# stoneMo/DeepAVFusion

Measured on AMD Instinct MI355X. Metric: AV-pairs/sec, DeepAVFusion ViT-B pre-training step (224px + 10s audio, image mask 0.75), higher is better.
Workload: dtype bf16; 1 GPU; AVMAE(DeepAVFusion base) fwd+bwd+allreduce+AdamW, B=64/GPU, 224x224 RGB + (128,640) log-mel, masks 0.75/0.8, fusion attn_ratio 0.25 mlp_ratio 1.0; global_batch=64, parallelism=dp1, graph=True

## Files before the change

deepavfusion_amd/_lib.py:

```python
from __future__ import annotations

import ctypes as C
import os

import torch

_HERE = os.path.dirname(os.path.abspath(__file__))
LIB_PATH = os.path.join(_HERE, 'libdavfusion_hip.so')

_p, _i, _l, _f, _sz = C.c_void_p, C.c_int, C.c_long, C.c_float, C.c_size_t

ABI_VERSION = 9

SIGNATURES = {
    'dav_abi_version': [],
    'dav_build_flags': [],
    'dav_last_error_string': [],
    'dav_tune': [_i, _i],
    'dav_gemm_nt_bf16': [_p, _p, _i, _i, _i, _i, _i, _p, _p, _i, _p, _i, _p, _i, _p, _p, _p, _i, _i, _p, _p, _i, _i, _i, _f, _i, _p],
    'dav_gemm_nt_ln_bf16': [_p, _p, _i, _i, _i, _i, _i, _p, _p, _i, _p, _i, _p, _i, _p, _p, _p, _i, _i, _p, _p, _i, _i, _i, _f, _i, _p, _p],
    'dav_ln_fold_grouped': [_p, _i, _p],
    'dav_rowstats_cast': [_p, _l, _i, _i, _i, _p, _p, _p],
    'dav_layernorm_bwd_twin': [_p, _l, _p, _i, _p, _l, _p, _i, _i, _i, _f, _p, _p, _p, _p,
                               _p, _l, _i, _p, _l, _p, _l,
# ... 51 lines not shown
    'dav_attn_bias_fwd_f32': [_p, _p, _p, _p, _p, _i, _i, _i, _i, _i, _i, _l, _i, _l, _i, _l, _i, _l, _i, _f, _p, _i, _i, _p],
    'dav_attn_bias_bwd_f32': [_p] * 10 + [_i] * 6 + [_l, _i] * 8 + [_f, _p, _i, _i, _p, _i, _p],
    'dav_attn_drop_fwd_f32': [_p, _p, _p, _p, _p, _i, _i, _i, _i, _i, _i, _l, _i, _l, _i, _l, _i, _l, _i, _f, _p, _i, _f, _p],
    'dav_attn_drop_bwd_f32': [_p] * 10 + [_i] * 6 + [_l, _i] * 8 + [_f, _p, _i, _f, _i, _p],
    'dav_patch_gather_f32': [_p, _i, _i, _i, _i, _i, _i, _p, _i, _p, _p],
    'dav_rows_gather_f32': [_p, _l, _i, _p, _i, _i, _i, _p, _l, _p],
    'dav_pair_expand_f32': [_p, _p, _i, _i, _i, _i, _p, _p],
    'dav_pair_reduce_f32': [_p, _i, _i, _i, _i, _p, _p, _p],
    'dav_patch_mse_bwd_f32': [_p, _p, _p, _p, _p, _p, _p, _i, _i, _i, _i, _p, _p],
    'dav_add_f32': [_p, _p, _p, _l, _p],
    'dav_logmel': [_p, _i, _i, _i, _i, _i, _p, _p, _p, _p, _p, _p, _f, _i, _i, _p, _p],
    'dav_log10_eps': [_p, _f, _l, _p, _p],
    'dav_mean_l2n_f32': [_p, _i, _i, _i, _l, _l, _p, _p],
    'dav_knn_topk_f32': [_p] * 6 + [_i, _i, _i, _i, _l, _l, _i, _i, _i, _p, _p, _p, _sz, _p],
    'dav_knn_topk_wide_f32': [_p] * 6 + [_i, _i, _i, _i, _l, _l, _i, _i, _i, _p, _p, _p, _sz, _p],
    'dav_knn_vote_f32': [_p, _p, _i, _i, _i, _i, _p, _p, _i, _i, _p, _i, _p, _p, _p],
    'dav_ap_auc_f64': [_p, _l, _i, _i, _i, _p, _l, _l, _p, _p, _p, _i, _p, _p, _p, _p, _sz, _p],
    'dav_frame_transform_u8': [_p, _i, _i, _i, _p, _i, _f, _f, _f, _f, _f, _f, _p, _p],
    'dav_wave_resample_tile': [_i, _i, _i],
    'dav_wave_resample': [_p, _i, _i, _i, _l, _p, _i, _i, _i, _p, _i, _p, _i, _l, _p],
    'dav_stft_c32': [_p, _i, _i, _l, _i, _i, _p, _p, _p, _p, _l, _p],
    'dav_istft_c32': [_p, _l, _i, _i, _i, _i, _p, _p, _p, _p, _l, _p],
    'dav_sep_mask_istft': [_p, _i, _i, _l, _p, _i, _i, _i, _i, _i, _p, _p, _p, _p, _p, _p, _p, _l, _p],
    'dav_batch_begin': [_i],
    'dav_batch_lane': [],
    'dav_batch_region': [_i],
    'dav_batch_skip': [_i],
    'dav_batch_suspend': [_i],
    'dav_batch_end': [],
    'dav_batch_abort': [],
    'dav_batch_stats': [_p, _p],
    'dav_adamw_flat': [_p, _p, _p, _p, _p, _l, _p, _p, _i, _f, _f, _f, _p, _f, _p, _i, _p, _p, _p],
    'dav_step_guard': [_p, _p, _p, _f, _f, _p, _p, _p],
    'dav_cast_transpose_grouped': [_p, _i, _p],
}

class DavLnReduce(C.Structure):
    _fields_ = [('workspace', C.c_void_p), ('dgamma', C.c_void_p), ('dbeta', C.c_void_p), ('rows', C.c_int), ('D', C.c_int)]


class DavNtLn(C.Structure):
    _fields_ = [('stats', C.c_void_p), ('stats2', C.c_void_p), ('A2', C.c_void_p), ('ln_c', C.c_void_p), ('eps', C.c_float),
                ('a_r0', C.c_int), ('a_r1', C.c_int), ('stats_out', C.c_void_p), ('twin_out', C.c_void_p), ('ld_twin', C.c_int)]


class DavLnFold(C.Structure):
# ... 76 lines not shown
```

deepavfusion_amd/autograd_bridge.py:

```python
from __future__ import annotations

import os

import torch

from . import engine as E
from . import ops
from .ops import F32


_SIDE_STREAMS = {}


def _streams(dev):
    main = torch.cuda.current_stream(dev)
    if os.environ.get('DAV_STREAMS', '1') == '0':
        return main, main, main
    key = dev.index if dev.index is not None else torch.cuda.current_device()
    if key not in _SIDE_STREAMS:
        _SIDE_STREAMS[key] = (torch.cuda.Stream(dev), torch.cuda.Stream(dev))
    sa, sf = _SIDE_STREAMS[key]
    return main, sa, sf


# ... 187 lines not shown


def encoder_bwd(enc, t, dxi_b=None, dxa_b=None, dxf_b=None, dxi32=None, dxa32=None, dxf32=None, layer_cb=None):
    with E.deferred_wgrads():
        _encoder_bwd(enc, t, dxi_b, dxa_b, dxf_b, dxi32, dxa32, dxf32, layer_cb)


def _encoder_bwd(enc, t, dxi_b, dxa_b, dxf_b, dxi32, dxa32, dxf32, layer_cb=None):
    B = t['B']
    dev = t['x_i'].device
    vis = _vis(enc)

    def final_norm(norm, x, st, dy_b, dy32):
        g = torch.empty_like(x)
        gb = torch.empty(x.shape, dtype=E.BF16, device=dev)
        if dy_b is None and dy32 is None:
            return g.zero_(), gb.zero_()
        E.ln_bwd(norm, None, x, B, st, dy_bf16=dy_b, dy_f32=dy32, dx1=g, dx1_bf16=gb)
        return g, gb
    g_i, g_ib = final_norm(vis.norm, t['x_i'], t['st_i'], dxi_b, dxi32)
    g_a, g_ab = final_norm(enc.audio.norm, t['x_a'], t['st_a'], dxa_b, dxa32)
    g_f, g_fb = final_norm(enc.fusion_norm, t['x_f'], t['st_f'], dxf_b, dxf32)
    blocks = list(zip(vis.blocks, enc.audio.blocks, enc.fusion_blocks))
    main, sa, sf = _streams(dev)
    batched = t['lanes']
    for l, ((bi, ba, fb), (ti, ta, tf)) in reversed(list(enumerate(zip(blocks, t['layers'])))):
        hold = (g_i, g_ib, g_a, g_ab, g_f, g_fb)
        if batched:
            dx_f = dx_i = dx_a = None
            lane_f = fb is not None and E.fusion_block_batchable(fb, tf.get('dp'), tf.get('dr')) and not E.FUSION_ON_STREAM
            if fb is not None and E.FUSION_ON_STREAM:
                sf.wait_stream(main)
                with torch.cuda.stream(sf):
                    dx_f, dx_i, dx_a = E.fusion_block_bwd(fb, tf, g_f, g_fb)
            elif fb is not None and not lane_f:
                dx_f, dx_i, dx_a = E.fusion_block_bwd(fb, tf, g_f, g_fb)
            idle = E.FUSION_IDLE_BWD if lane_f else 0
            with E.batch() as bt:
                bt.lane()
                st_i = E.block_bwd_head(bi, ti, g_i, g_ib, idle_before_attn=idle)
                bt.lane()
                st_a = E.block_bwd_head(ba, ta, g_a, g_ab, idle_before_attn=idle)
                if lane_f:
                    bt.lane()
                    dx_f, dx_i, dx_a = E.fusion_block_bwd(fb, tf, g_f, g_fb)
            acc = 1 if fb is not None else 0
# ... 13 lines not shown
            with torch.cuda.stream(sa):
                g_a, g_ab, _ = E.block_bwd(ba, ta, g_a, g_ab)
            g_i, g_ib, _ = E.block_bwd(bi, ti, g_i, g_ib)
            main.wait_stream(sa)
        else:
            sa.wait_stream(main)
            sf.wait_stream(main)
            with torch.cuda.stream(sf):
                dx_f, dx_i, dx_a = E.fusion_block_bwd(fb, tf, g_f, g_fb)
            with torch.cuda.stream(sa):
                g_a, g_ab, dxf_a = E.block_bwd(ba, ta, g_a, g_ab, dx_mod=dx_a, dx_mod_acc=1,
                                               before_ln1=lambda: sa.wait_stream(sf))
            g_i, g_ib, dx_f = E.block_bwd(bi, ti, g_i, g_ib, dx_fus=dx_f, dx_fus_acc=1, dx_mod=dx_i, dx_mod_acc=1,
                                          before_ln1=lambda: main.wait_stream(sf))
            main.wait_stream(sa)
            main.wait_stream(sf)
            if sa is main:
                g_f, g_fb = dx_f.add_(dxf_a), None
            elif _ADD_CAST and E.PRECISION != 'fp32' and dx_f.is_contiguous() and dxf_a.is_contiguous() and dx_f.numel() % 4 == 0:
                g_f, g_fb = ops.add_cast(dx_f, dxf_a)
            else:
                g_f, g_fb = dx_f + dxf_a, None
        del hold
        if E.wgrad_flush_due(l, len(blocks)):
            E.flush_wgrads()
        if layer_cb is not None and l > 0:
            layer_cb(l)
    E.patch_embed_bwd(vis, t['t_pi'], g_i, g_ib)
    E.patch_embed_bwd(enc.audio, t['t_pa'], g_a, g_ab)
    E.gbuf(enc.fusion_tokens).add_(g_f.sum(dim=0, keepdim=True))
    E._ready(enc.fusion_tokens)


class _EncoderFn(torch.autograd.Function):
    @staticmethod
    def forward(ctx, enc, image, audio, ik32, ak32, return_embs, need_tape, *params):
        ctx.set_materialize_grads(False)
        with E.ln_fuse_for(need_tape):
            _, f32s, embs, tape = encoder_fwd(enc, image, audio, ik32, ak32, want_f32=True, collect_embs=return_embs)
        ctx.enc, ctx.tape = enc, (tape if need_tape else None)
        B = image.shape[0]
        outs = [x.view(B, -1, x.shape[-1]) for x in f32s]
        flat_embs = [e for tri in embs for e in tri]
        ctx.mark_non_differentiable(*flat_embs)
        return (*outs, *flat_embs)

    @staticmethod
    def backward(ctx, gi, ga, gf, *_):
        if ctx.tape is None:
            raise RuntimeError('backward through DeepAVFusion.forward called without a saved tape')
        c = lambda g: None if g is None else g.contiguous().view(-1, g.shape[-1])
        encoder_bwd(ctx.enc, ctx.tape, dxi32=c(gi), dxa32=c(ga), dxf32=c(gf))
        ctx.tape = None
# ... 111 lines not shown

    @staticmethod
    def backward(ctx, g):
        with E.deferred_wgrads():
            dx_f, dx_i, dx_a = E.fusion_block_bwd(ctx.fb, ctx.tape, g.contiguous(), None)
        return (None, dx_f, dx_i, dx_a) + (None,) * ctx.np


def fusion_block(fb, xmm, xv, xa):
    c = lambda x: x.to(dtype=F32).contiguous()
    return _FusionBlockFn.apply(fb, c(xmm), c(xv), c(xa), *list(fb.parameters()))


def avmae_fwd(model, image, audio, noise_i, noise_a):
    with E.fold_scope(model):
        return _avmae_fwd(model, image, audio, noise_i, noise_a)


def _avmae_fwd(model, image, audio, noise_i, noise_a):
    enc = model.encoder
    B = image.shape[0]
    Li, La = model.image_gs[0] * model.image_gs[1], model.audio_gs[0] * model.audio_gs[1]
    nki, nka = int(Li * (1 - model.image_mask_ratio)), int(La * (1 - model.audio_mask_ratio))
    ik, im, ir, ik32, ir32 = ops.mask_build(noise_i, nki)
    ak, am, ar, ak32, ar32 = ops.mask_build(noise_a, nka)
    (xi_b, xa_b, xf_b), _, _, t_enc = encoder_fwd(enc, image, audio, ik32, ak32)
    nF = enc.fusion_tokens.shape[1]
    dec_i, dec_a = model.decoder('image'), model.decoder('audio')
    main, sa, _ = _streams(image.device)
    lanes = t_enc['lanes']
    if lanes:
        with E.batch() as bt:
            bt.lane()
            pred_i, t_di = E.decoder_fwd(dec_i, xi_b, xf_b, ir32, B, nki, nF)
            loss_i, t_li = E.loss_fwd(image, pred_i, im, model.image_norm_loss)
            bt.lane()
            pred_a, t_da = E.decoder_fwd(dec_a, xa_b, xf_b, ar32, B, nka, nF)
            loss_a, t_la = E.loss_fwd(audio, pred_a, am, model.audio_norm_loss)
    else:
        si = main
        sa.wait_stream(main)
        if si is not main:
            si.wait_stream(main)

        def chain(dec, x_b, r32, nk, target, mask, norm_loss):
            pred, t_d = yield from E.decoder_fwd_steps(dec, x_b, xf_b, r32, B, nk, nF)
            loss, t_l = E.loss_fwd(target, pred, mask, norm_loss)
            return pred, t_d, loss, t_l
# ... 42 lines not shown
                if g_p is not None:
                    dp = (dp.float() + g_p.reshape(dp.shape)).to(E.BF16)
                return (yield from E.decoder_bwd_steps(dec, t_d, dp, k32, B))
            (dxa_b, dxf_a), (dxi_b, dxf_i) = paired_steps(
                chain(dec_a, t['audio'], t['pred_a'], t['am'], t['t_la'], g_la, g_pa, t['t_da'], t['ak32']), sa,
                chain(dec_i, t['image'], t['pred_i'], t['im'], t['t_li'], g_li, g_pi, t['t_di'], t['ik32']), si, DEC_JOIN)
            main.wait_stream(sa)
            if si is not main:
                main.wait_stream(si)
            E.deferred_operands_to(main)
    else:
        sa.wait_stream(main)
        with torch.cuda.stream(sa), E.deferred_wgrads():
            dpa = E.loss_bwd(t['audio'], t['pred_a'], t['am'], t['t_la'], g_la)
            if g_pa is not None:
                dpa = (dpa.float() + g_pa.reshape(dpa.shape)).to(E.BF16)
            dxa_b, dxf_a = E.decoder_bwd(dec_a, t['t_da'], dpa, t['ak32'], B)
        with E.deferred_wgrads():
            dpi = E.loss_bwd(t['image'], t['pred_i'], t['im'], t['t_li'], g_li)
            if g_pi is not None:
                dpi = (dpi.float() + g_pi.reshape(dpi.shape)).to(E.BF16)
            dxi_b, dxf_i = E.decoder_bwd(dec_i, t['t_di'], dpi, t['ik32'], B)
        main.wait_stream(sa)
    dxf32 = dxf_i.float() + dxf_a.float()
    if layer_cb is not None:
        layer_cb(len(model.encoder.fusion_blocks))
    encoder_bwd(model.encoder, t['t_enc'], dxi_b=dxi_b, dxa_b=dxa_b, dxf32=dxf32, layer_cb=layer_cb)


class _AVMAEFn(torch.autograd.Function):
    @staticmethod
    def forward(ctx, model, image, audio, noise_i, noise_a, need_tape, *params):
        ctx.set_materialize_grads(False)
        with E.ln_fuse_for(need_tape):
            outs, tape, aux = avmae_fwd(model, image, audio, noise_i, noise_a)
        ctx.model, ctx.tape, ctx.np = model, (tape if need_tape else None), len(params)
        model._last_masks = aux
        return outs

    @staticmethod
    def backward(ctx, g_li, g_la, g_pi, g_pa):
        z = lambda g: g.contiguous() if g is not None else torch.zeros((), dtype=F32, device=ctx.tape['image'].device)
        avmae_bwd(ctx.model, ctx.tape, z(g_li), z(g_la), g_pi, g_pa)
        ctx.tape = None
        return (None,) * (6 + ctx.np)


# ... 13 lines not shown
```

deepavfusion_amd/engine.py:

```python
from __future__ import annotations

import os
from typing import Callable, Dict, List, NamedTuple, Optional

import torch

from . import ops
from .ops import F32

BF16 = torch.bfloat16
PRECISION = 'bf16'


def set_precision(p: str):
    global BF16, PRECISION
    if p not in ('bf16', 'fp32'):
        raise ValueError(p)
    PRECISION = p
    BF16 = torch.float32 if p == 'fp32' else torch.bfloat16

_GRAD_READY: Optional[Callable[[torch.nn.Parameter], None]] = None


def set_grad_ready_hook(fn: Optional[Callable[[torch.nn.Parameter], None]]):
    global _GRAD_READY
    _GRAD_READY = fn


def _ready(*params):
    if _GRAD_READY is not None:
        if _BATCH is not None:
            _BATCH.pending_ready.extend(params)
            return
        for p in params:
            if p is not None and p.requires_grad:
                _GRAD_READY(p)


_BATCH = None
BATCH_STATS = [0, 0]

BATCH_POLICY = {'1': 'on', '0': 'off'}.get(os.environ.get('DAV_BATCH', ''), 'auto')
LANE_MIN_ROWS = int(os.environ.get('DAV_LANE_MIN_ROWS', str(1 << 30)))
FUSION_ON_STREAM = os.environ.get('DAV_FUSION_STREAM', '1') != '0'


def set_batch_policy(policy: str):
    global BATCH_POLICY
    assert policy in ('on', 'off', 'auto')
    BATCH_POLICY = policy


def batching_allowed() -> bool:
    return BATCH_POLICY != 'off' and PRECISION == 'bf16'


def lanes_for(rows: int) -> bool:
    if not batching_allowed():
        return False
    return BATCH_POLICY == 'on' or rows >= LANE_MIN_ROWS


class batch:
    def __init__(self, auto_lanes: bool = False):
        self.auto_lanes = auto_lanes
        self.active = False
        self.pending_ready = []
# ... 1290 lines not shown
    A = _e((B * nk, K), BF16, img.device)
    ops.patch_gather(img, ids_keep32, nk, A, pt)
    Wb = wcache(pe.proj.weight)
    tok = _e((B, nk, D), F32, img.device)
    pos_by_id = ids_keep32 is not None and not clip
    if ln_fuse_ok(D) and K % 64 == 0:
        tw = (_e((B * nk, D), BF16, img.device), _e((B * nk, D // 64, 2), F32, img.device))
        ops.gemm_nt_ln(A, Wb, B * nk, D, K, prod=dict(stats_out=tw[1], twin_out=tw[0], ld_twin=D), bias=pe.proj.bias, res=vit.pos_embed,
                       ldres=D, res_rows=ids_keep32 if pos_by_id else None, res_rowmap=None if pos_by_id else (L, 0, 0), C_out=tok)
        tw_set(tok, *tw)
    else:
        ops.gemm_nt(A, Wb, B * nk, D, K, bias=pe.proj.bias, res=vit.pos_embed, ldres=D,
                    res_rows=ids_keep32 if pos_by_id else None, res_rowmap=None if pos_by_id else (L, 0, 0), C_out=tok)
    return tok, dict(A=A, nk=nk)


def patch_embed_bwd(vit, t, g, gb):
    pe = vit.patch_embed
    D = vit.embed_dim
    A = t['A']
    M, K = A.shape
    if gb is None:
        gb = to_bf16(g)
    ops.gemm_tn(gb, A, M, D, K, gbuf(pe.proj.weight).view(D, K), beta=1, bias_grad=gbuf(pe.proj.bias))
    _ready(pe.proj.weight, pe.proj.bias)


def drain(steps):
    try:
        while True:
            next(steps)
    except StopIteration as e:
        return e.value


def decoder_fwd(dec, x_b, xf_b, ids_restore32, B, nk, nF):
    return drain(decoder_fwd_steps(dec, x_b, xf_b, ids_restore32, B, nk, nF))


def decoder_fwd_steps(dec, x_b, xf_b, ids_restore32, B, nk, nF):
    L = ids_restore32.shape[1]
    Dd = dec.embed.weight.shape[0]
    dev = x_b.device
    emb = lin_fwd(dec.embed, x_b, B * nk)
    x = _e((B, nF + L, Dd), F32, dev)
    lin_fwd(dec.embed, xf_b, B * nF, out=x, c_rowmap=(nF, nF + L, 0))
# ... 16 lines not shown
        return pred.view(B, L, P), tape
    hN = _e((B * L, D_), BF16, dev)
    mean, rstd = _e((B * L,), F32, dev), _e((B * L,), F32, dev)
    xs = x.view(-1)[nF * Dd:]
    ops.layernorm_fwd(xs, (nF + L) * Dd, L, None, 0, 0, B, Dd, dec.norm.weight, dec.norm.bias, dec.norm.eps, hN, None, mean, rstd)
    pred = lin_fwd(dec.pred, hN, B * L)
    P = pred.shape[1]
    tape = dict(x_b=x_b, xf_b=xf_b, x_last=x, tapes=tapes, hN=hN, stN=(mean, rstd), ids_restore32=ids_restore32, nk=nk, nF=nF, L=L)
    return pred.view(B, L, P), tape


def decoder_bwd(dec, t, dpred_b, ids_keep32, B):
    return drain(decoder_bwd_steps(dec, t, dpred_b, ids_keep32, B))


def decoder_bwd_steps(dec, t, dpred_b, ids_keep32, B):
    nk, nF, L = t['nk'], t['nF'], t['L']
    Dd = dec.embed.weight.shape[0]
    dev = dpred_b.device
    fused = t.get('ln_fused', False)
    dhN = lin_bwd(dec.pred, dpred_b, None if fused else t['hN'], B * L, wgrad=not fused)
    g = _e((B, nF + L, Dd), F32, dev)
    gb = _e((B * (nF + L), Dd), BF16, dev)
    g[:, :nF].zero_()
    gb.view(B, nF + L, Dd)[:, :nF].zero_()
    if fused:
        xb, st = t['tw_last']
        hN = _e((B * L, Dd), BF16, dev)
        ops.layernorm_bwd_twin((xb, nF * Dd), (nF + L) * Dd, (st, nF * (Dd // 64) * 2), L, None, 0, None, 0, B, Dd, dec.norm.eps,
                               dhN, None, dec.norm.weight, dec.norm.bias,
                               (g, nF * Dd), (nF + L) * Dd, 0, None, 0, (gb, nF * Dd), (nF + L) * Dd,
                               h_out=hN, dgamma=gbuf(dec.norm.weight), dbeta=gbuf(dec.norm.bias))
        lin_wgrad(dec.pred, dpred_b, hN, B * L)
    else:
        xs = t['x_last'].view(-1)[nF * Dd:]
        ops.layernorm_bwd(xs, (nF + L) * Dd, L, None, 0, 0, B, Dd, dhN, None, dec.norm.weight, t['stN'][0], t['stN'][1],
                          g.view(-1)[nF * Dd:], (nF + L) * Dd, 0, None, 0, gb.view(-1)[nF * Dd:], (nF + L) * Dd,
                          None, 0, 0, None, 0, None, 0, gbuf(dec.norm.weight), gbuf(dec.norm.bias))
    _ready(dec.norm.weight, dec.norm.bias)
    swin = getattr(dec, 'arch', 'plain') == 'swin'
    yield
    for blk, bt in zip(reversed(list(dec.blocks)), reversed(t['tapes'])):
        if swin:
            g, gb = swin_block_bwd(blk, bt, g, gb)
        else:
            g, gb, _ = block_bwd(blk, bt, g, gb)
        yield
    d_emb = _e((B * nk, Dd), BF16, dev)
    d_embf = _e((B * nF, Dd), BF16, dev)
    ops.rows_gather_cast(g, (nF + L) * Dd, nF, ids_keep32, B, nk, Dd, d_emb)
    ops.rows_gather_cast(g, (nF + L) * Dd, 0, None, B, nF, Dd, d_embf)
    ops.unshuffle_bwd_reduce(g, (nF + L) * Dd, nF, t['ids_restore32'], B, L, nk, Dd, gbuf(dec.pos_embed), gbuf(dec.mask_token))
    _ready(dec.pos_embed, dec.mask_token)
    dx_b = lin_bwd(dec.embed, d_emb, t['x_b'], B * nk, final=False)
    dxf_b = lin_bwd(dec.embed, d_embf, t['xf_b'], B * nF)
    return dx_b, dxf_b


LOG2E = 1.4426950408889634


def swin_block_fwd(blk, x, nF):
    B, R, D = x.shape
    L, dev = R - nF, x.device
    heads, nW = blk.num_heads, blk.num_windows
    A = blk.attn.window_area
    N, hd, M, Mw = A + nF, D // heads, B * R, B * nW * (A + nF)
    h1, _, st1 = ln_fwd(blk.norm1, None, x, B)
    seq = _e((Mw, D), BF16, dev)
    ops.window_unfold(h1, blk.rows32, B, nW, A, nF, L, D, 1.0, seq)
    qkv = lin_fwd(blk.attn.qkv, seq, Mw, out_bf16=True)
    nb = nW if blk.attn_mask is not None else 1
    ld = (N + 31) // 32 * 32
    bias = _e((nb, heads, N, ld), F32, dev)
    ops.relpos_bias_build(blk.attn.relative_position_bias_table, blk.index32, blk.attn_mask, nb, heads, A, N, ld,
# ... 35 lines not shown
    ops.relpos_bias_bwd(dS, blk.index32, B * nW, heads, A, N, t['ld'], table.shape[0], gbuf(table))
    _ready(table)
    dseq = lin_bwd(blk.attn.qkv, dqkv, t['seq'], Mw, dx_bf16=False)
    dh1 = _e((M, D), F32, dev)
    ops.window_fold(dseq, blk.inv32, None, B, nW, A, nF, L, D, 1.0, dh1)
    dx = _e((B, R, D), F32, dev)
    dxb = _e((M, D), BF16, dev)
    ln_bwd(blk.norm1, None, x, B, t['st1'], dy_f32=dh1, dx1=dx, res1=g1, dx1_bf16=dxb)
    return dx, dxb


def loss_fwd(img, pred, mask, norm_pix):
    B, L = mask.shape
    dev = img.device
    lp, tm, tr = _e((B * L,), F32, dev), _e((B * L,), F32, dev), _e((B * L,), F32, dev)
    loss, msum = _e((1,), F32, dev), _e((1,), F32, dev)
    ops.patch_mse_fwd(img, pred, mask, norm_pix, lp, tm, tr, loss, msum)
    return loss.view(()), dict(tm=tm, tr=tr, msum=msum)


def loss_bwd(img, pred, mask, t, gout):
    B, L, P = pred.shape
    dpred = _e((B * L, P), BF16, img.device)
    ops.patch_mse_bwd(img, pred, mask, t['tm'], t['tr'], t['msum'], gout, dpred)
    return dpred
```

deepavfusion_amd/ops.py:

```python
from __future__ import annotations

import ctypes as C
from typing import Optional, Sequence

import torch

from . import _lib

BF16 = torch.bfloat16
F32 = torch.float32


def _stream():
    return torch.cuda.current_stream().cuda_stream


import threading

_TLS = threading.local()


def hold(*tensors):
    h = getattr(_TLS, 'hold', None)
    if h is not None:
# ... 409 lines not shown

def unshuffle_bwd_reduce(dx, dx_bs, row_off, ids_restore32, B, L, nk, D, dpos, dmask_token):
    lib = _lib.load()
    _lib.check(lib.dav_unshuffle_bwd_reduce(_ptr(dx), dx_bs, row_off, _ptr(ids_restore32), B, L, nk, D, _ptr(dpos),
                                            _ptr(dmask_token), _stream()), 'dav_unshuffle_bwd_reduce')


def patch_mse_fwd(img, pred, mask, norm_pix, loss_patch, tmean, trstd, loss, mask_sum):
    lib = _lib.load()
    B, Cc, H, W = img.shape
    _lib.check(lib.dav_patch_mse_fwd(_ptr(img), _ptr(pred), _ptr(mask), B, Cc, H, W, int(norm_pix), _ptr(loss_patch),
                                     _ptr(tmean), _ptr(trstd), _ptr(loss), _ptr(mask_sum), _stream()), 'dav_patch_mse_fwd')


def patch_mse_bwd(img, pred, mask, tmean, trstd, mask_sum, gout, dpred_bf16):
    lib = _lib.load()
    B, Cc, H, W = img.shape
    if dpred_bf16.dtype == F32:
        _lib.check(lib.dav_patch_mse_bwd_f32(_ptr(img), _ptr(pred), _ptr(mask), _ptr(tmean), _ptr(trstd), _ptr(mask_sum), _ptr(gout),
                                             B, Cc, H, W, _ptr(dpred_bf16), _stream()), 'dav_patch_mse_bwd_f32')
        return
    _lib.check(lib.dav_patch_mse_bwd(_ptr(img), _ptr(pred), _ptr(mask), _ptr(tmean), _ptr(trstd), _ptr(mask_sum), _ptr(gout),
                                     B, Cc, H, W, _ptr(dpred_bf16), _stream()), 'dav_patch_mse_bwd')


def pair_expand(Pv, Pa, B, nv, na, Wd, out):
    lib = _lib.load()
    if out.dtype == F32:
        _lib.check(lib.dav_pair_expand_f32(_ptr(Pv), _ptr(Pa), B, nv, na, Wd, _ptr(out), _stream()), 'dav_pair_expand_f32')
        return
    _lib.check(lib.dav_pair_expand(_ptr(Pv), _ptr(Pa), B, nv, na, Wd, _ptr(out), _stream()), 'dav_pair_expand')


def pair_reduce(d, B, nv, na, Wd, dPv, dPa):
    lib = _lib.load()
    if d.dtype == F32:
        _lib.check(lib.dav_pair_reduce_f32(_ptr(d), B, nv, na, Wd, _ptr(dPv), _ptr(dPa), _stream()), 'dav_pair_reduce_f32')
        return
    _lib.check(lib.dav_pair_reduce(_ptr(d), B, nv, na, Wd, _ptr(dPv), _ptr(dPa), _stream()), 'dav_pair_reduce')


def cast_bf16(x, y):
    lib = _lib.load()
    _lib.check(lib.dav_cast_bf16(_ptr(x), _ptr(y), x.numel(), _stream()), 'dav_cast_bf16')


# ... 379 lines not shown
```

include/dav_kernels.h:

```cpp
#ifndef DAV_KERNELS_H_
#define DAV_KERNELS_H_

#include <stddef.h>
#include <stdint.h>

#ifdef __HIPCC__
#include <hip/hip_runtime.h>
#else
typedef struct ihipStream_t* hipStream_t;
#endif

#ifdef __cplusplus
extern "C" {
#endif

#define DAV_ABI_VERSION 9
int dav_abi_version(void);
int dav_build_flags(void);
const char* dav_last_error_string(void);
int dav_tune(int knob, int value);

int dav_gemm_nt_bf16(const void* A, const void* B, int M, int N, int K, int lda, int ldb, const int* a_rowmap,
                     const float* bias, int act, const void* aux, int ldaux, const float* res, int ldres,
                     const int* res_rowmap, const int* res_rows, void* C, int ldc, int c_is_bf16, const int* c_rowmap,
// ... 195 lines not shown
int dav_attn_bias_bwd_f32(const float* Q, const float* K, const float* V, const float* O, const float* dO, const float* LSE,
                          float* Delta, float* dQ, float* dK, float* dV, int B, int H, int Nq, int Nk, int dqk, int dv, long q_bs,
                          int q_rs, long k_bs, int k_rs, long v_bs, int v_rs, long o_bs, int o_rs, long do_bs, int do_rs,
                          long dq_bs, int dq_rs, long dk_bs, int dk_rs, long dv_bs, int dv_rs, float scale, const float* bias,
                          int bias_nb, int bias_ld, float* dS, int part, hipStream_t stream);
int dav_attn_drop_fwd_f32(const float* Q, const float* K, const float* V, float* O, float* LSE, int B, int H, int Nq, int Nk,
                          int dqk, int dv, long q_bs, int q_rs, long k_bs, int k_rs, long v_bs, int v_rs, long o_bs, int o_rs,
                          float scale, const void* keep, int keep_ld, float keep_scale, hipStream_t stream);
int dav_attn_drop_bwd_f32(const float* Q, const float* K, const float* V, const float* O, const float* dO, const float* LSE,
                          float* Delta, float* dQ, float* dK, float* dV, int B, int H, int Nq, int Nk, int dqk, int dv, long q_bs,
                          int q_rs, long k_bs, int k_rs, long v_bs, int v_rs, long o_bs, int o_rs, long do_bs, int do_rs,
                          long dq_bs, int dq_rs, long dk_bs, int dk_rs, long dv_bs, int dv_rs, float scale, const void* keep,
                          int keep_ld, float keep_scale, int part, hipStream_t stream);
int dav_patch_gather_f32(const float* img, int B, int C, int T, int H, int W, int pt, const int* ids_keep32, int nk, float* A,
                         hipStream_t stream);
int dav_rows_gather_f32(const float* x, long x_bs, int row_off, const int* ids32, int B, int n, int D, float* out, long out_bs,
                        hipStream_t stream);
int dav_pair_expand_f32(const float* Pv, const float* Pa, int B, int nv, int na, int Wd, float* out, hipStream_t stream);
int dav_pair_reduce_f32(const float* d, int B, int nv, int na, int Wd, float* dPv, float* dPa, hipStream_t stream);
int dav_patch_mse_bwd_f32(const float* img, const float* pred, const float* mask, const float* tmean, const float* trstd,
                          const float* mask_sum, const float* gout, int B, int C, int H, int W, float* dpred, hipStream_t stream);
int dav_add_f32(const float* a, const float* b, float* out, long n, hipStream_t stream);

int dav_batch_begin(int auto_lanes);
int dav_batch_lane(void);
int dav_batch_region(int begin);
int dav_batch_skip(int steps);
int dav_batch_suspend(int on);
int dav_batch_end(void);
int dav_batch_abort(void);
int dav_batch_stats(int* recorded_ops, int* issued_launches);

#ifdef __cplusplus
}
#endif
#endif
```

Before: 2659 AV-pairs/s.

## Add fused seam kernels for masks, loss bwd, reductions, zeroing and patch-embed wgrad

Adds a set of small HIP kernels behind a DAV_SEAMS switch, on by default for bf16. Mask building for image and audio now runs as one launch. It also adds a vectorized loss gradient, a decoder unshuffle reduction with unrolled batch loads, a bf16+bf16→f32 add and a batch-sum accumulate for the fusion tokens. The zeroing of two rows becomes a single kernel, and the patch-embed backward moves into the layer loop as deferred wgrad. These target launch count and small memory-bound kernels around the main encoder/decoder. In exchange they add atomics and deferred wgrad ordering that could change numerics or the schedule.

```diff
diff --git a/deepavfusion_amd/_lib.py b/deepavfusion_amd/_lib.py
--- a/deepavfusion_amd/_lib.py
+++ b/deepavfusion_amd/_lib.py
@@ -97,6 +97,12 @@
     'dav_stft_c32': [_p, _i, _i, _l, _i, _i, _p, _p, _p, _p, _l, _p],
     'dav_istft_c32': [_p, _l, _i, _i, _i, _i, _p, _p, _p, _p, _l, _p],
     'dav_sep_mask_istft': [_p, _i, _i, _l, _p, _i, _i, _i, _i, _i, _p, _p, _p, _p, _p, _p, _p, _l, _p],
+    'dav_unshuffle_bwd_reduce2': [_p, _l, _i, _p, _i, _i, _i, _i, _p, _p, _p],
+    'dav_patch_mse_bwd2': [_p, _p, _p, _p, _p, _p, _p, _i, _i, _i, _i, _p, _p],
+    'dav_mask_build_pair': [_p, _i, _i, _i, _p, _p, _p, _p, _p] * 2 + [_p],
+    'dav_add2_bf16_f32': [_p, _p, _p, _l, _p],
+    'dav_batch_sum_acc': [_p, _l, _i, _l, _p, _p],
+    'dav_rows_zero_pair': [_p, _p, _i, _i, _i, _i, _p],
     'dav_batch_begin': [_i],
     'dav_batch_lane': [],
     'dav_batch_region': [_i],
diff --git a/deepavfusion_amd/autograd_bridge.py b/deepavfusion_amd/autograd_bridge.py
--- a/deepavfusion_amd/autograd_bridge.py
+++ b/deepavfusion_amd/autograd_bridge.py
@@ -233,6 +233,7 @@
     g_a, g_ab = final_norm(enc.audio.norm, t['x_a'], t['st_a'], dxa_b, dxa32)
     g_f, g_fb = final_norm(enc.fusion_norm, t['x_f'], t['st_f'], dxf_b, dxf32)
     blocks = list(zip(vis.blocks, enc.audio.blocks, enc.fusion_blocks))
+    pembed_queued = False
     main, sa, sf = _streams(dev)
     batched = t['lanes']
     for l, ((bi, ba, fb), (ti, ta, tf)) in reversed(list(enumerate(zip(blocks, t['layers'])))):
@@ -292,13 +293,22 @@
             else:
                 g_f, g_fb = dx_f + dxf_a, None
         del hold
+        if l == 0 and E.seam('pembed'):
+            E.patch_embed_bwd(vis, t['t_pi'], g_i, g_ib)
+            E.patch_embed_bwd(enc.audio, t['t_pa'], g_a, g_ab)
+            pembed_queued = True
         if E.wgrad_flush_due(l, len(blocks)):
             E.flush_wgrads()
         if layer_cb is not None and l > 0:
             layer_cb(l)
-    E.patch_embed_bwd(vis, t['t_pi'], g_i, g_ib)
-    E.patch_embed_bwd(enc.audio, t['t_pa'], g_a, g_ab)
-    E.gbuf(enc.fusion_tokens).add_(g_f.sum(dim=0, keepdim=True))
+    if not pembed_queued:
+        E.patch_embed_bwd(vis, t['t_pi'], g_i, g_ib)
+        E.patch_embed_bwd(enc.audio, t['t_pa'], g_a, g_ab)
+    ft = E.gbuf(enc.fusion_tokens)
+    if E.seam('fsum') and g_f.dtype == F32 and g_f.is_contiguous() and ft.is_contiguous() and ft.numel() % 4 == 0 and g_f.numel() == B * ft.numel():
+        ops.batch_sum_acc(g_f, ft.numel(), B, ft.numel(), ft)
+    else:
+        ft.add_(g_f.sum(dim=0, keepdim=True))
     E._ready(enc.fusion_tokens)
 
 
@@ -456,8 +466,11 @@
     B = image.shape[0]
     Li, La = model.image_gs[0] * model.image_gs[1], model.audio_gs[0] * model.audio_gs[1]
     nki, nka = int(Li * (1 - model.image_mask_ratio)), int(La * (1 - model.audio_mask_ratio))
-    ik, im, ir, ik32, ir32 = ops.mask_build(noise_i, nki)
-    ak, am, ar, ak32, ar32 = ops.mask_build(noise_a, nka)
+    if E.seam('mask'):
+        (ik, im, ir, ik32, ir32), (ak, am, ar, ak32, ar32) = ops.mask_build_pair(noise_i, nki, noise_a, nka)
+    else:
+        ik, im, ir, ik32, ir32 = ops.mask_build(noise_i, nki)
+        ak, am, ar, ak32, ar32 = ops.mask_build(noise_a, nka)
     (xi_b, xa_b, xf_b), _, _, t_enc = encoder_fwd(enc, image, audio, ik32, ak32)
     nF = enc.fusion_tokens.shape[1]
     dec_i, dec_a = model.decoder('image'), model.decoder('audio')
@@ -546,7 +559,11 @@
                 dpi = (dpi.float() + g_pi.reshape(dpi.shape)).to(E.BF16)
             dxi_b, dxf_i = E.decoder_bwd(dec_i, t['t_di'], dpi, t['ik32'], B)
         main.wait_stream(sa)
-    dxf32 = dxf_i.float() + dxf_a.float()
+    if (E.seam('add2') and dxf_i.dtype == E.BF16 and dxf_a.dtype == E.BF16 and dxf_i.is_contiguous() and dxf_a.is_contiguous()
+            and dxf_i.numel() % 4 == 0):
+        dxf32 = ops.add2_bf16_f32(dxf_i, dxf_a)
+    else:
+        dxf32 = dxf_i.float() + dxf_a.float()
     if layer_cb is not None:
         layer_cb(len(model.encoder.fusion_blocks))
     encoder_bwd(model.encoder, t['t_enc'], dxi_b=dxi_b, dxa_b=dxa_b, dxf32=dxf32, layer_cb=layer_cb)
diff --git a/deepavfusion_amd/csrc/step/seams.hip b/deepavfusion_amd/csrc/step/seams.hip
--- /dev/null
+++ b/deepavfusion_amd/csrc/step/seams.hip
@@ -0,0 +1,272 @@
+#include "common.h"
+#include "dav_kernels.h"
+
+namespace {
+
+__device__ __forceinline__ void add4(float4& s, const float4& v) { s.x += v.x; s.y += v.y; s.z += v.z; s.w += v.w; }
+
+constexpr int UB = 8;
+
+__global__ __launch_bounds__(256) void unshuffle_bwd_reduce2_kernel(const float* dx, long dx_bs, int row_off, const int* restore,
+                                                                    int B, int L, int nk, int D, float* dpos, float* dmask_token) {
+  __shared__ float4 part[4][64];
+  const int lane = threadIdx.x & 63, w = threadIdx.x >> 6;
+  const int nch = D >> 2;
+  const int c = blockIdx.x * 64 + lane;
+  const int r = blockIdx.y * 4 + w;
+  const bool live = r < L && c < nch;
+  float4 sp = float4{0.f, 0.f, 0.f, 0.f}, sm = sp;
+  if (live) {
+    const float4* src = reinterpret_cast<const float4*>(dx + (long)(row_off + r) * D) + c;
+    const long bs4 = dx_bs >> 2;
+    const int* rs = restore + r;
+    int b = 0;
+    for (; b + UB <= B; b += UB) {
+      float4 v[UB];
+      int j[UB];
+#pragma unroll
+      for (int u = 0; u < UB; ++u) { v[u] = src[(b + u) * bs4]; j[u] = rs[(long)(b + u) * L]; }
+#pragma unroll
+      for (int u = 0; u < UB; ++u) {
+        add4(sp, v[u]);
+        if (j[u] >= nk) add4(sm, v[u]);
+      }
+    }
+    for (; b < B; ++b) {
+      const float4 v = src[b * bs4];
+      add4(sp, v);
+      if (rs[(long)b * L] >= nk) add4(sm, v);
+    }
+    float4* dp = reinterpret_cast<float4*>(dpos + (long)r * D) + c;
+    float4 o = *dp;
+    add4(o, sp);
+    *dp = o;
+  }
+  part[w][lane] = sm;
+  __syncthreads();
+  if (w == 0 && c < nch) {
+    float4 t = part[0][lane];
+    add4(t, part[1][lane]); add4(t, part[2][lane]); add4(t, part[3][lane]);
+    float* dm = dmask_token + 4 * c;
+    unsafeAtomicAdd(dm + 0, t.x); unsafeAtomicAdd(dm + 1, t.y); unsafeAtomicAdd(dm + 2, t.z); unsafeAtomicAdd(dm + 3, t.w);
+  }
+}
+
+template <int C>
+__device__ __forceinline__ const float* patch_px(const float* img, int b, int l, int H, int W, int lane) {
+  const int gW = W >> 4, gy = l / gW, gx = l % gW;
+  return img + (((long)b * C) * H + gy * 16 + (lane >> 2)) * W + gx * 16 + (lane & 3) * 4;
+}
+
+template <int C>
+__global__ __launch_bounds__(256) void patch_mse_bwd2_kernel(const float* img, const float* pred, const float* mask, const float* tmean,
+                                                             const float* trstd, const float* mask_sum, const float* gout, int B, int H,
+                                                             int W, bf16_t* dpred) {
+  constexpr int P = 256 * C;
+  const int lane = threadIdx.x & 63;
+  const int gw = (blockIdx.x * blockDim.x + threadIdx.x) >> 6, nwaves = (gridDim.x * blockDim.x) >> 6;
+  const int L = (H >> 4) * (W >> 4), n = B * L;
+  const long plane = (long)H * W;
+  const float coef = (gout ? gout[0] : 1.f) * 2.f / (P * mask_sum[0]);
+  for (int row = gw; row < n; row += nwaves) {
+    const float m = mask[row] * coef;
+    uint2* dst = reinterpret_cast<uint2*>(dpred + (long)row * P + lane * 4 * C);
+    if (m == 0.f) {
+#pragma unroll
+      for (int k = 0; k < C; ++k) dst[k] = uint2{0u, 0u};
+      continue;
+    }
+    const float mean = tmean[row], rstd = trstd[row];
+    const float* tp = patch_px<C>(img, row / L, row % L, H, W, lane);
+    const float4* pp = reinterpret_cast<const float4*>(pred + (long)row * P + lane * 4 * C);
+    float4 t[C], p4[C];
+#pragma unroll
+    for (int c = 0; c < C; ++c) { t[c] = *reinterpret_cast<const float4*>(tp + c * plane); p4[c] = pp[c]; }
+    const float* p = reinterpret_cast<const float*>(p4);
+    float g[4 * C];
+#pragma unroll
+    for (int c = 0; c < C; ++c) {
+      const float tc[4] = {t[c].x, t[c].y, t[c].z, t[c].w};
+#pragma unroll
+      for (int j = 0; j < 4; ++j) g[j * C + c] = m * (p[j * C + c] - (tc[j] - mean) * rstd);
+    }
+#pragma unroll
+    for (int k = 0; k < C; ++k) dst[k] = uint2{pack2bf(g[4 * k], g[4 * k + 1]), pack2bf(g[4 * k + 2], g[4 * k + 3])};
+  }
+}
+
+struct MaskSide {
+  const float* noise;
+  int64_t* ids_keep;
+  int64_t* ids_restore;
+  float* mask;
+  int* ids_keep32;
+  int* ids_restore32;
+  int N, L, P, len_keep;
+};
+
+__global__ __launch_bounds__(1024) void mask_build_pair_kernel(MaskSide sa, MaskSide sb) {
+  extern __shared__ __attribute__((aligned(16))) char smem[];
+  const bool first = (int)blockIdx.x < sa.N;
+  const MaskSide& s = first ? sa : sb;
+  const int row = first ? blockIdx.x : blockIdx.x - sa.N;
+  const int L = s.L, P = s.P, len_keep = s.len_keep;
+  float* key = reinterpret_cast<float*>(smem);
+  int* idx = reinterpret_cast<int*>(smem + (size_t)P * 4);
+  const int tid = threadIdx.x, nt = blockDim.x;
+  for (int i = tid; i < P; i += nt) {
+    key[i] = i < L ? s.noise[(long)row * L + i] : __int_as_float(0x7f800000);
+    idx[i] = i;
+  }
+  __syncthreads();
+  for (int k = 2; k <= P; k <<= 1) {
+    for (int j = k >> 1; j > 0; j >>= 1) {
+      for (int i = tid; i < P; i += nt) {
+        const int ixj = i ^ j;
+        if (ixj > i) {
+          const float a = key[i], b = key[ixj];
+          const int ia = idx[i], ib = idx[ixj];
+          const bool a_gt_b = (a > b) || (a == b && ia > ib);
+          const bool up = (i & k) == 0;
+          if (a_gt_b == up) { key[i] = b; key[ixj] = a; idx[i] = ib; idx[ixj] = ia; }
+        }
+      }
+      __syncthreads();
+    }
+  }
+  for (int i = tid; i < L; i += nt) {
+    const int src = idx[i];
+    s.ids_restore[(long)row * L + src] = i;
+    s.ids_restore32[(long)row * L + src] = i;
+    s.mask[(long)row * L + src] = i < len_keep ? 0.f : 1.f;
+    if (i < len_keep) {
+      s.ids_keep[(long)row * len_keep + i] = src;
+      s.ids_keep32[(long)row * len_keep + i] = src;
+    }
+  }
+}
+
+__global__ __launch_bounds__(256) void add2_bf16_f32_kernel(const uint2* a, const uint2* b, float4* out, long n4) {
+  for (long i = (long)blockIdx.x * blockDim.x + threadIdx.x; i < n4; i += (long)gridDim.x * blockDim.x) {
+    const uint2 x = a[i], y = b[i];
+    out[i] = float4{__uint_as_float(x.x << 16) + __uint_as_float(y.x << 16),
+                    __uint_as_float(x.x & 0xffff0000u) + __uint_as_float(y.x & 0xffff0000u),
+                    __uint_as_float(x.y << 16) + __uint_as_float(y.y << 16),
+                    __uint_as_float(x.y & 0xffff0000u) + __uint_as_float(y.y & 0xffff0000u)};
+  }
+}
+
+__global__ __launch_bounds__(64) void batch_sum_acc_kernel(const float* x, long x_bs, int B, long n4, float* acc) {
+  const long i = (long)blockIdx.x * blockDim.x + threadIdx.x;
+  if (i >= n4) return;
+  const float4* src = reinterpret_cast<const float4*>(x) + i;
+  const long bs4 = x_bs >> 2;
+  float4 s = float4{0.f, 0.f, 0.f, 0.f};
+  int b = 0;
+  for (; b + UB <= B; b += UB) {
+    float4 v[UB];
+#pragma unroll
+    for (int u = 0; u < UB; ++u) v[u] = src[(b + u) * bs4];
+#pragma unroll
+    for (int u = 0; u < UB; ++u) add4(s, v[u]);
+  }
+  for (; b < B; ++b) add4(s, src[b * bs4]);
+  float4* dst = reinterpret_cast<float4*>(acc) + i;
+  float4 o = *dst;
+  add4(o, s);
+  *dst = o;
+}
+
+__global__ __launch_bounds__(256) void rows_zero_pair_kernel(float* g, void* gb, int B, long bs, long z) {
+  const long per = (z >> 2) + (z >> 3), total = (long)B * per;
+  for (long i = (long)blockIdx.x * blockDim.x + threadIdx.x; i < total; i += (long)gridDim.x * blockDim.x) {
+    const long b = i / per, k = i % per;
+    if (k < (z >> 2)) reinterpret_cast<float4*>(g + b * bs)[k] = float4{0.f, 0.f, 0.f, 0.f};
+    else reinterpret_cast<uint4*>((bf16_t*)gb + b * bs)[k - (z >> 2)] = uint4{0u, 0u, 0u, 0u};
+  }
+}
+
+int wave_grid(long rows) {
+  long g = (rows + 3) / 4;
+  return (int)(g > 2048 ? 2048 : (g < 1 ? 1 : g));
+}
+
+int flat_grid(long items) {
+  long g = (items + 255) / 256;
+  return (int)(g > 4096 ? 4096 : (g < 1 ? 1 : g));
+}
+
+bool mis(const void* p, unsigned mask) { return ((uintptr_t)p & mask) != 0; }
+
+int mask_side(MaskSide& s, const float* noise, int N, int L, int len_keep, int64_t* ids_keep, int64_t* ids_restore, float* mask,
+              int* ids_keep32, int* ids_restore32) {
+  if (N <= 0 || L <= 0 || L > 4096 || len_keep < 0 || len_keep > L) return DAV_ERR_SHAPE;
+  int P = 1;
+  while (P < L) P <<= 1;
+  s = MaskSide{noise, ids_keep, ids_restore, mask, ids_keep32, ids_restore32, N, L, P, len_keep};
+  return DAV_OK;
+}
+
+}
+
+extern "C" int dav_unshuffle_bwd_reduce2(const float* dx, long dx_bs, int row_off, const int* ids_restore32, int B, int L, int nk,
+                                         int D, float* dpos, float* dmask_token, hipStream_t stream) {
+  if (B <= 0 || L <= 0 || D <= 0 || (D & 3) || row_off < 0 || dx_bs < 0) return DAV_ERR_SHAPE;
+  if ((dx_bs & 3) || mis(dx, 15) || mis(dpos, 15) || mis(dmask_token, 15) || mis(ids_restore32, 3)) return DAV_ERR_ALIGN;
+  const dim3 grid(((D >> 2) + 63) / 64, (L + 3) / 4);
+  DAV_LAUNCH(unshuffle_bwd_reduce2_kernel, grid, dim3(256), 0, stream, dx, dx_bs, row_off, ids_restore32, B, L, nk, D, dpos, dmask_token);
+  return dav_launch_status();
+}
+
+extern "C" int dav_patch_mse_bwd2(const float* img, const float* pred, const float* mask, const float* tmean, const float* trstd,
+                                  const float* mask_sum, const float* gout, int B, int C, int H, int W, void* dpred_bf16,
+                                  hipStream_t stream) {
+  if (B <= 0 || H <= 0 || W <= 0 || (H & 15) || (W & 15) || (C != 1 && C != 3)) return DAV_ERR_SHAPE;
+  const long rows = (long)B * (H >> 4) * (W >> 4);
+  if (rows > 0x7fffffffL) return DAV_ERR_SHAPE;
+  if (mis(img, 15) || mis(pred, 15) || mis(dpred_bf16, 7)) return DAV_ERR_ALIGN;
+  const dim3 grid(wave_grid(rows)), block(256);
+  if (C == 3) DAV_LAUNCH(patch_mse_bwd2_kernel<3>, grid, block, 0, stream, img, pred, mask, tmean, trstd, mask_sum, gout, B, H, W, (bf16_t*)dpred_bf16);
+  else DAV_LAUNCH(patch_mse_bwd2_kernel<1>, grid, block, 0, stream, img, pred, mask, tmean, trstd, mask_sum, gout, B, H, W, (bf16_t*)dpred_bf16);
+  return dav_launch_status();
+}
+
+extern "C" int dav_mask_build_pair(const float* noise_a, int Na, int La, int len_keep_a, int64_t* ids_keep_a, int64_t* ids_restore_a,
+                                   float* mask_a, int* ids_keep32_a, int* ids_restore32_a, const float* noise_b, int Nb, int Lb,
+                                   int len_keep_b, int64_t* ids_keep_b, int64_t* ids_restore_b, float* mask_b, int* ids_keep32_b,
+                                   int* ids_restore32_b, hipStream_t stream) {
+  MaskSide sa, sb;
+  if (mask_side(sa, noise_a, Na, La, len_keep_a, ids_keep_a, ids_restore_a, mask_a, ids_keep32_a, ids_restore32_a) != DAV_OK ||
+      mask_side(sb, noise_b, Nb, Lb, len_keep_b, ids_keep_b, ids_restore_b, mask_b, ids_keep32_b, ids_restore32_b) != DAV_OK)
+    return DAV_ERR_SHAPE;
+  const int P = sa.P > sb.P ? sa.P : sb.P;
+  const int nt = P / 2 < 64 ? 64 : (P / 2 > 1024 ? 1024 : P / 2);
+  DAV_LAUNCH(mask_build_pair_kernel, dim3(Na + Nb), dim3(nt), (size_t)P * 8, stream, sa, sb);
+  return dav_launch_status();
+}
+
+extern "C" int dav_add2_bf16_f32(const void* a_bf16, const void* b_bf16, float* out, long n, hipStream_t stream) {
+  if (n <= 0 || (n & 3)) return DAV_ERR_SHAPE;
+  if (mis(a_bf16, 15) || mis(b_bf16, 15) || mis(out, 15)) return DAV_ERR_ALIGN;
+  DAV_LAUNCH(add2_bf16_f32_kernel, dim3(flat_grid(n >> 2)), dim3(256), 0, stream, (const uint2*)a_bf16, (const uint2*)b_bf16,
+             (float4*)out, n >> 2);
+  return dav_launch_status();
+}
+
+extern "C" int dav_batch_sum_acc(const float* x, long x_bs, int B, long n, float* acc, hipStream_t stream) {
+  if (B <= 0 || n <= 0 || (n & 3) || x_bs < n) return DAV_ERR_SHAPE;
+  if ((x_bs & 3) || mis(x, 15) || mis(acc, 15)) return DAV_ERR_ALIGN;
+  const long n4 = n >> 2, g = (n4 + 63) / 64;
+  if (g > 0x7fffffffL) return DAV_ERR_SHAPE;
+  DAV_LAUNCH(batch_sum_acc_kernel, dim3((int)g), dim3(64), 0, stream, x, x_bs, B, n4, acc);
+  return dav_launch_status();
+}
+
+extern "C" int dav_rows_zero_pair(float* g, void* g_bf16, int B, int R, int nF, int D, hipStream_t stream) {
+  if (B <= 0 || R <= 0 || D <= 0 || nF <= 0 || nF > R) return DAV_ERR_SHAPE;
+  const long bs = (long)R * D, z = (long)nF * D;
+  if ((bs & 7) || (z & 7)) return DAV_ERR_SHAPE;
+  if (mis(g, 15) || mis(g_bf16, 15)) return DAV_ERR_ALIGN;
+  DAV_LAUNCH(rows_zero_pair_kernel, dim3(flat_grid((long)B * ((z >> 2) + (z >> 3)))), dim3(256), 0, stream, g, g_bf16, B, bs, z);
+  return dav_launch_status();
+}
diff --git a/deepavfusion_amd/engine.py b/deepavfusion_amd/engine.py
--- a/deepavfusion_amd/engine.py
+++ b/deepavfusion_amd/engine.py
@@ -43,6 +43,31 @@
 BATCH_POLICY = {'1': 'on', '0': 'off'}.get(os.environ.get('DAV_BATCH', ''), 'auto')
 LANE_MIN_ROWS = int(os.environ.get('DAV_LANE_MIN_ROWS', str(1 << 30)))
 FUSION_ON_STREAM = os.environ.get('DAV_FUSION_STREAM', '1') != '0'
+
+
+SEAM_PIECES = ('reduce', 'loss', 'mask', 'add2', 'fsum', 'zero', 'pembed')
+
+
+def _parse_seams(v):
+    if v in (True, None, '1', 'on', 'all'):
+        return frozenset(SEAM_PIECES)
+    if v in (False, '0', 'off', ''):
+        return frozenset()
+    pieces = frozenset(x.strip() for x in v.split(',')) if isinstance(v, str) else frozenset(v)
+    assert pieces <= set(SEAM_PIECES), sorted(pieces - set(SEAM_PIECES))
+    return pieces
+
+
+SEAMS = _parse_seams(os.environ.get('DAV_SEAMS', '1'))
+
+
+def set_seams(v):
+    global SEAMS
+    SEAMS = _parse_seams(v)
+
+
+def seam(piece: str) -> bool:
+    return piece in SEAMS and PRECISION == 'bf16'
 
 
 def set_batch_policy(policy: str):
@@ -1379,6 +1404,9 @@
     M, K = A.shape
     if gb is None:
         gb = to_bf16(g)
+    if seam('pembed') and _DEFERRED is not None and M % 64 == 0:
+        lin_wgrad(pe.proj, gb, A, M)
+        return
     ops.gemm_tn(gb, A, M, D, K, gbuf(pe.proj.weight).view(D, K), beta=1, bias_grad=gbuf(pe.proj.bias))
     _ready(pe.proj.weight, pe.proj.bias)
 
@@ -1441,8 +1469,11 @@
     dhN = lin_bwd(dec.pred, dpred_b, None if fused else t['hN'], B * L, wgrad=not fused)
     g = _e((B, nF + L, Dd), F32, dev)
     gb = _e((B * (nF + L), Dd), BF16, dev)
-    g[:, :nF].zero_()
-    gb.view(B, nF + L, Dd)[:, :nF].zero_()
+    if seam('zero') and nF > 0 and (nF * Dd) % 8 == 0 and (L * Dd) % 8 == 0:
+        ops.rows_zero_pair(g, gb, B, nF + L, nF, Dd)
+    else:
+        g[:, :nF].zero_()
+        gb.view(B, nF + L, Dd)[:, :nF].zero_()
     if fused:
         xb, st = t['tw_last']
         hN = _e((B * L, Dd), BF16, dev)
@@ -1469,7 +1500,8 @@
     d_embf = _e((B * nF, Dd), BF16, dev)
     ops.rows_gather_cast(g, (nF + L) * Dd, nF, ids_keep32, B, nk, Dd, d_emb)
     ops.rows_gather_cast(g, (nF + L) * Dd, 0, None, B, nF, Dd, d_embf)
-    ops.unshuffle_bwd_reduce(g, (nF + L) * Dd, nF, t['ids_restore32'], B, L, nk, Dd, gbuf(dec.pos_embed), gbuf(dec.mask_token))
+    reduce = ops.unshuffle_bwd_reduce2 if seam('reduce') and Dd % 4 == 0 else ops.unshuffle_bwd_reduce
+    reduce(g, (nF + L) * Dd, nF, t['ids_restore32'], B, L, nk, Dd, gbuf(dec.pos_embed), gbuf(dec.mask_token))
     _ready(dec.pos_embed, dec.mask_token)
     dx_b = lin_bwd(dec.embed, d_emb, t['x_b'], B * nk, final=False)
     dxf_b = lin_bwd(dec.embed, d_embf, t['xf_b'], B * nF)
@@ -1551,5 +1583,6 @@
 def loss_bwd(img, pred, mask, t, gout):
     B, L, P = pred.shape
     dpred = _e((B * L, P), BF16, img.device)
-    ops.patch_mse_bwd(img, pred, mask, t['tm'], t['tr'], t['msum'], gout, dpred)
+    bwd = ops.patch_mse_bwd2 if seam('loss') and dpred.dtype == torch.bfloat16 else ops.patch_mse_bwd
+    bwd(img, pred, mask, t['tm'], t['tr'], t['msum'], gout, dpred)
     return dpred
diff --git a/deepavfusion_amd/ops.py b/deepavfusion_amd/ops.py
--- a/deepavfusion_amd/ops.py
+++ b/deepavfusion_amd/ops.py
@@ -455,6 +455,54 @@
         return
     _lib.check(lib.dav_patch_mse_bwd(_ptr(img), _ptr(pred), _ptr(mask), _ptr(tmean), _ptr(trstd), _ptr(mask_sum), _ptr(gout),
                                      B, Cc, H, W, _ptr(dpred_bf16), _stream()), 'dav_patch_mse_bwd')
+
+
+def unshuffle_bwd_reduce2(dx, dx_bs, row_off, ids_restore32, B, L, nk, D, dpos, dmask_token):
+    lib = _lib.load()
+    _lib.check(lib.dav_unshuffle_bwd_reduce2(_ptr(dx), dx_bs, row_off, _ptr(ids_restore32), B, L, nk, D, _ptr(dpos),
+                                             _ptr(dmask_token), _stream()), 'dav_unshuffle_bwd_reduce2')
+
+
+def patch_mse_bwd2(img, pred, mask, tmean, trstd, mask_sum, gout, dpred_bf16):
+    lib = _lib.load()
+    B, Cc, H, W = img.shape
+    _lib.check(lib.dav_patch_mse_bwd2(_ptr(img), _ptr(pred), _ptr(mask), _ptr(tmean), _ptr(trstd), _ptr(mask_sum), _ptr(gout),
+                                      B, Cc, H, W, _ptr(dpred_bf16), _stream()), 'dav_patch_mse_bwd2')
+
+
+def mask_build_pair(noise_a, len_keep_a, noise_b, len_keep_b):
+    lib = _lib.load()
+    args, outs = [], []
+    for noise, len_keep in ((noise_a, len_keep_a), (noise_b, len_keep_b)):
+        N, L = noise.shape
+        dev = noise.device
+        ids_keep = torch.empty(N, len_keep, dtype=torch.int64, device=dev)
+        ids_restore = torch.empty(N, L, dtype=torch.int64, device=dev)
+        mask = torch.empty(N, L, dtype=F32, device=dev)
+        ids_keep32 = torch.empty(N, len_keep, dtype=torch.int32, device=dev)
+        ids_restore32 = torch.empty(N, L, dtype=torch.int32, device=dev)
+        args += [_ptr(noise.contiguous()), N, L, len_keep, _ptr(ids_keep), _ptr(ids_restore), _ptr(mask), _ptr(ids_keep32), _ptr(ids_restore32)]
+        outs.append((ids_keep, mask, ids_restore, ids_keep32, ids_restore32))
+    _lib.check(lib.dav_mask_build_pair(*args, _stream()), 'dav_mask_build_pair')
+    return outs[0], outs[1]
+
+
+def add2_bf16_f32(a, b, out=None):
+    lib = _lib.load()
+    if out is None:
+        out = torch.empty(a.shape, dtype=F32, device=a.device)
+    _lib.check(lib.dav_add2_bf16_f32(_ptr(a), _ptr(b), _ptr(out), a.numel(), _stream()), 'dav_add2_bf16_f32')
+    return out
+
+
+def batch_sum_acc(x, x_bs, B, n, acc):
+    lib = _lib.load()
+    _lib.check(lib.dav_batch_sum_acc(_ptr(x), x_bs, B, n, _ptr(acc), _stream()), 'dav_batch_sum_acc')
+
+
+def rows_zero_pair(g, g_bf16, B, R, nF, D):
+    lib = _lib.load()
+    _lib.check(lib.dav_rows_zero_pair(_ptr(g), _ptr(g_bf16), B, R, nF, D, _stream()), 'dav_rows_zero_pair')
 
 
 def pair_expand(Pv, Pa, B, nv, na, Wd, out):
diff --git a/include/dav_kernels.h b/include/dav_kernels.h
--- a/include/dav_kernels.h
+++ b/include/dav_kernels.h
@@ -241,6 +241,18 @@
                           const float* mask_sum, const float* gout, int B, int C, int H, int W, float* dpred, hipStream_t stream);
 int dav_add_f32(const float* a, const float* b, float* out, long n, hipStream_t stream);
 
+int dav_unshuffle_bwd_reduce2(const float* dx, long dx_bs, int row_off, const int* ids_restore32, int B, int L, int nk, int D,
+                              float* dpos, float* dmask_token, hipStream_t stream);
+int dav_patch_mse_bwd2(const float* img, const float* pred, const float* mask, const float* tmean, const float* trstd,
+                       const float* mask_sum, const float* gout, int B, int C, int H, int W, void* dpred_bf16, hipStream_t stream);
+int dav_mask_build_pair(const float* noise_a, int Na, int La, int len_keep_a, int64_t* ids_keep_a, int64_t* ids_restore_a,
+                        float* mask_a, int* ids_keep32_a, int* ids_restore32_a, const float* noise_b, int Nb, int Lb,
+                        int len_keep_b, int64_t* ids_keep_b, int64_t* ids_restore_b, float* mask_b, int* ids_keep32_b,
+                        int* ids_restore32_b, hipStream_t stream);
+int dav_add2_bf16_f32(const void* a_bf16, const void* b_bf16, float* out, long n, hipStream_t stream);
+int dav_batch_sum_acc(const float* x, long x_bs, int B, long n, float* acc, hipStream_t stream);
+int dav_rows_zero_pair(float* g, void* g_bf16, int B, int R, int nF, int D, hipStream_t stream);
+
 int dav_batch_begin(int auto_lanes);
 int dav_batch_lane(void);
 int dav_batch_region(int begin);
```

Result: no change. 2676 AV-pairs/s (median of 6 runs) (+0.6%).
